# farshid83/dpsvm

Measured on AMD Instinct MI355X. Metric: wall-clock training time (s) to tol=1e-3, MNIST even-odd RBF, at 1/2/4/8 MI355X, lower is better.
Workload: dtype fp32

## Files before the change

### dpsvm_amd/csrc/include/dpsvm/device_state.hpp

```cpp
#pragma once

#include <cstdint>

namespace dpsvm {

constexpr int kNQ = 16;
constexpr int kStepRows = 128;
constexpr int kStepThreads = 256;
constexpr int kFinThreads = 1024;
constexpr int kRowsKC = 1008;

enum CacheMode : int32_t {
  kCacheDense = 0,
  kCacheLRU = 1,
};

enum RowOp : int32_t {
  kOpCompute = 0,
  kOpFetch = 1,
};

enum DoneCode : int32_t {
  kRunning = 0,
  kConverged = 1,
// ... 64 lines not shown
      if (r.when(f)) return *out = r.kind, true;
  return false;
}

inline int ws_new_auto(int ws_new, int q, int dp) {
  const int n = ws_new > 0 ? (ws_new < q ? ws_new : q) : (dp >= 128 ? q : 3 * q / 4);
  return n > 2 ? n : 2;
}

struct alignas(16) SmoCtrl {
  int32_t iter;
  int32_t done;
  int32_t final_applied;
  int32_t nq;
  int32_t i_hi, i_lo;
  int32_t line_hi, line_lo;
  float c_hi, c_lo;
  float b_hi, b_lo;
  int32_t n_compute;
  int32_t n_spill;
  int32_t q_idx[kNQ];
  int32_t q_line[kNQ];
  int32_t q_op[kNQ];
  int32_t q_hsrc[kNQ];
  int32_t q_hspill[kNQ];
  float q_sq[kNQ];
  const float* q_ptr[kNQ];
  int32_t hand, hhand, pad0, pad1;
  int64_t hits, misses, rows_computed, x_passes, spec_rows, host_hits, spills;
};

struct alignas(16) SmoStatus {
  int64_t iter;
  int32_t done;
  int32_t seq;
  float b_hi, b_lo;
  int64_t hits, misses, rows_computed, x_passes, spec_rows, host_hits, spills;
  int64_t outer;
  int64_t ws_p1_round;
  int32_t ws_p, ws_damped;
  float nu_ext[4];
};

struct alignas(16) CandRecord {
  uint64_t key_hi, key_lo;
};

struct alignas(16) FusedRec {
  int32_t i_hi, i_lo;
  float a_hi, a_lo;
  int32_t iter, done;
  float b_hi, b_lo;
};
struct alignas(16) FusedCacheRec {
  int32_t i_hi, i_lo;
  float a_hi, a_lo;
  int32_t iter, done;
  float b_hi, b_lo;
  int32_t n_new;
  int32_t hand0, span;
  int32_t hand;
  int32_t hit_line[2];
  int32_t hhand, pad0;
  int32_t line[kNQ];
  int32_t key[kNQ];
  int32_t old[kNQ];
  int32_t hline[kNQ];
  int32_t hold[kNQ];
  int64_t hits, misses, rows_computed, x_passes, spec_rows, host_hits, spills;
};

constexpr int kFusedThreads = 256;
constexpr int kStatusEvery = 32;

struct SmoArgs {
  const float* x;
  const float* xsq;
  const float* y;
  float* alpha;
  float* f;
  float* lines;
  int64_t ldl;
  int32_t* slot_of;
  int32_t* key_of;
  uint8_t* ref;
  float* hlines;
  int32_t* hslot_of;
  int32_t* hkey_of;
  int32_t H;
  uint64_t* partials;
  SmoCtrl* ctrl;
  SmoStatus* status;
  const uint8_t* records;
  uint8_t* my_record;
  int64_t rec_bytes;
  int64_t n, nl, off;
  int64_t x_row0;
  int32_t d, dp, G, L;
  int32_t world;
  int32_t cache_mode;
  int32_t partitioned;
  int32_t spec;
  int32_t clip;
  float C, gamma, eps, tau;
  int64_t max_iter;
  int32_t fused_rows;
  int32_t fused_G;
  uint64_t* stamps;
  int32_t* plru_meta;
  int64_t plru_stride;
  uint64_t* const* xpeer;
  int32_t xrank, xworld;
  int32_t xstride;
  int32_t xpoll_kb;
  int32_t xpoll_sleep;
  int64_t xtimeout_ticks;
  int32_t* census;
  int64_t census_ticks;
  int32_t eta_gram;
};
constexpr int kXchGranules = 4;

constexpr int kWsMax = 192;
constexpr int kWsCand = 16;
constexpr int kWsCandStd = 8;
constexpr int kWsCand1 = 4;
constexpr int kWsSelThreads = 256;
constexpr int kWsMaxGroups = 256;
constexpr int kWsListsPerThread = 4;
constexpr int kWsMaxRPT = 32;
constexpr int kWsSolveThreads = 1024;
constexpr int64_t kWsAutoRows = 50000;
constexpr int kWsMaxBlocks = 128;
constexpr int kWsAutoBlocks = 32;
constexpr int kWsAutoUnion = 16 * kWsMax;
constexpr int kWsMaxAll = 32 * kWsMax;
constexpr int kWsCacheWindow = 512;

inline int64_t ws_cache_min_lines(int q_max) { return 2 * (int64_t)q_max + kWsCacheWindow; }
constexpr int kWsWindowMulti = 8192;
inline int64_t ws_cache_multi_min_lines(int blocks, int q) { return 2 * (int64_t)blocks * q + kWsWindowMulti; }

inline int64_t production_line_cap(int64_t cache_lines, int ws_q, int engines) {
  if (cache_lines <= 0 || engines != 0) return cache_lines;
  const int64_t lo = ws_cache_min_lines(ws_q);
  return cache_lines < lo ? lo : cache_lines;
}
constexpr int kWsMergeThreads = 1024;
constexpr int kWsMaxPass1Splits = 16;
constexpr int kWsPass1Cols = 1024;
constexpr int64_t kWsAutoBlocksRows = 50000;
constexpr int64_t kWsSwitchRounds = 32;

struct alignas(16) WsCtrl {
  int64_t iter;
  int64_t outer;
  int32_t done;
  int32_t n_apply;
  int32_t q[2];
  float b_hi, b_lo;
  int32_t nonfinite;
  int32_t n_miss;
  int32_t hand;
  int32_t solve_cnt;
  int32_t rank_cnt;
  int32_t pad[1];
  int32_t idx[2][kWsMaxAll];
  int32_t line[2][kWsMaxAll];
  int32_t apply_idx[kWsMaxAll];
  int32_t apply_line[kWsMaxAll];
  float apply_coef[kWsMaxAll];
  int32_t miss_row[kWsMaxAll], miss_line[kWsMaxAll];
  int64_t rows_computed, row_hits;
  int32_t uidx[2][kWsMaxAll];
  int32_t uq[2];
  int32_t qb[2][kWsMaxBlocks];
  int32_t nab[kWsMaxBlocks];
  int32_t inb[kWsMaxBlocks];
  int32_t badb[kWsMaxBlocks];
  int32_t pad2[3];
  float t_last;
  int32_t n_damped;
  int32_t p_act;
  int32_t p_round;
  int32_t clipb[kWsMaxBlocks];
  int64_t p1_round;
  int32_t nu_cls;
  int32_t pad3[3];
  float nu_ext[4];
};

struct WsArgs {
  const float* gram;
  int64_t ldg;
  const float* y;
  float* alpha;
  float* f;
  int64_t n, nl, off;
  int32_t G, rpt;
  int32_t world;
  int32_t G_all;
  int32_t q_max, n_new, inner_max;
  float rel_local;
  float eps_floor;
  float C, eps, tau;
  int32_t clip;
  int64_t max_iter;
  int32_t cache;
  int32_t L;
  int32_t* slot_of;
  int32_t* key_of;
  uint64_t* cand_out;
  uint64_t* cand;
  float* subg;
  float* aux;
  WsCtrl* ctrl;
  SmoStatus* status;
  uint64_t* stamps;
  uint64_t* const* xpeer;
  int32_t xrank;
  int32_t xcw;
  int64_t xsub;
  int64_t xsub_rows;
  int64_t xpart;
  int64_t xtimeout_ticks;
  int32_t blocks;
  float* dfs;
  float* dalpha;
  double* part;
  int32_t rank;
  int32_t aux_stride;
  int32_t wss;
  float t_halve;
  int32_t clip_fallback;
  int32_t ks;
  int32_t p1G;
  uint64_t* sorted;
  int32_t direct_sub;
  int32_t ncand;
  const float* c_row;
  int64_t fold;
  int32_t diag;
  int32_t nu_mode;
};
constexpr int ws_ncand(int ncand) { return ncand > 0 && ncand < kWsCand ? ncand : kWsCand; }
constexpr int64_t ws_xch_words(int64_t G_all, int64_t q_max) {
  return 2 * G_all * 4 * kWsCand1 + 2 * q_max * (q_max + 1);
}
constexpr int64_t ws_xch_cand_words_multi(int64_t G_all) { return 2 * G_all * 4 * kWsCand; }
constexpr int64_t ws_xch_part_words(int64_t P1_all, int64_t ks) { return 2 * P1_all * ks * 4; }
constexpr int64_t ws_xch_sub_words(int64_t P, int64_t q, int64_t q1) {
  return 2 * ((P * q * (q + 1)) > (q1 * (q1 + 1)) ? P * q * (q + 1) : q1 * (q1 + 1));
}
constexpr int64_t ws_xch_words_multi(int64_t G_all, int64_t P1_all, int64_t ks, int64_t P, int64_t q, int64_t q1) {
  return ws_xch_cand_words_multi(G_all) + ws_xch_part_words(P1_all, ks) + ws_xch_sub_words(P, q, q1);
}
constexpr int kStampRing = 4096;
constexpr int kStampSlots = 12;

}
```

### dpsvm_amd/csrc/kernels/ws_common.hpp

```cpp
#pragma once

#include <hip/hip_runtime.h>

#include "dpsvm/common.hpp"
#include "dpsvm/device_state.hpp"
#include "device_util.hpp"
#include "xch.hpp"

namespace dpsvm {
namespace dev {

constexpr int kWsGatherThreads = 256;
constexpr int kWsMaxCand = kWsMaxGroups * kWsCand1;
constexpr int kWsHash = 1024;

#define WS_STAMP(k)                                                                            \
  do {                                                                                         \
    if (a.stamps) a.stamps[(size_t)(c->outer % kStampRing) * 2 * kStampSlots + (k)] =          \
        __builtin_amdgcn_s_memrealtime();                                                      \
  } while (0)

__device__ __forceinline__ float f_add1(float fj, float c, float k) {
#pragma clang fp contract(off)
  return fj + c * k;
// ... 83 lines not shown
  return bin;
}

__device__ __forceinline__ uint64_t block_scan_fields(uint64_t v, uint64_t* wsum, uint64_t* total) {
  const int lane = threadIdx.x & 63, wave = threadIdx.x >> 6;
  const uint64_t below = (1ull << lane) - 1ull;
  uint64_t pre = 0, wtot = 0;
#pragma unroll
  for (int f = 0; f < 4; ++f) {
#pragma unroll
    for (int b = 0; b < 3; ++b) {
      const int bit = 12 * f + b;
      const uint64_t mk = __ballot((v >> bit) & 1);
      pre += (uint64_t)__popcll(mk & below) << bit;
      wtot += (uint64_t)__popcll(mk) << bit;
    }
  }
  if (lane == 0) wsum[wave] = wtot;
  __syncthreads();
  uint64_t off = 0, tot = 0;
#pragma unroll
  for (int w = 0; w < kWsGatherThreads / 64; ++w) {
    off += w < wave ? wsum[w] : 0;
    tot += wsum[w];
  }
  *total = tot;
  __syncthreads();
  return off + pre;
}

__device__ __forceinline__ uint32_t ws_hash(int32_t idx) { return ((uint32_t)idx * 2654435761u) >> 22; }

__device__ __forceinline__ void ws_hash_insert(int32_t* keys, int32_t* vals, int32_t idx, int32_t v) {
  uint32_t h = ws_hash(idx);
  while (true) {
    const int32_t old = atomicCAS(keys + h, -1, idx);
    if (old == -1) {
      vals[h] = v;
      return;
    }
    h = (h + 1) & (kWsHash - 1);
  }
}

__device__ __forceinline__ int32_t ws_hash_find(const int32_t* keys, const int32_t* vals, int32_t idx) {
  uint32_t h = ws_hash(idx);
  for (int probe = 0; probe < kWsHash; ++probe) {
    const int32_t k = keys[h];
    if (k == idx) return vals[h];
    if (k == -1) return -1;
    h = (h + 1) & (kWsHash - 1);
  }
  return -1;
}

__device__ __forceinline__ void ws_status(SmoStatus* s, const WsCtrl* c) {
  if (!s) return;
  s->iter = c->iter;
  s->done = c->done;
  s->b_hi = c->b_hi;
  s->b_lo = c->b_lo;
  s->outer = c->outer;
  s->rows_computed = c->rows_computed;
  s->misses = c->rows_computed;
  s->hits = c->row_hits;
  s->ws_p1_round = c->p1_round;
  s->ws_p = c->p_act;
  s->ws_damped = c->n_damped;
  __atomic_store_n(&s->seq, (int32_t)c->outer, __ATOMIC_RELEASE);
}

__device__ __forceinline__ int64_t ws_xcand(const WsArgs& a, int par, int slot) {
  return ((int64_t)par * a.G_all + slot) * a.xcw;
}

__device__ __forceinline__ int64_t ws_xrow(const WsArgs& a, int par, int row) {
  return a.xsub + ((int64_t)par * a.xsub_rows + row) * (a.q_max + 1);
}

__device__ __forceinline__ int64_t ws_nparts(const WsArgs& a) {
  return (int64_t)a.world * a.p1G * max(1, a.ks);
}
__device__ __forceinline__ int64_t ws_xpart(const WsArgs& a, int par, int64_t k) {
  return a.xpart + ((int64_t)par * ws_nparts(a) + k) * 4;
}

__device__ __forceinline__ bool ws_tag_ok(uint64_t g, uint64_t t) { return (g >> 48) == (t >> 48); }

__device__ __forceinline__ void ws_put64(uint64_t* dst, uint64_t t, uint64_t v) {
  xch_store<true>(dst, t | (v >> 16));
  xch_store<true>(dst + 1, t | (v & 0xffffull));
}
__device__ __forceinline__ uint64_t ws_get64(uint64_t g0, uint64_t g1) {
  return ((g0 & ((1ull << 48) - 1)) << 16) | (g1 & 0xffffull);
}

template <int N>
__device__ __forceinline__ bool ws_poll(const WsArgs& a, const uint64_t* g, uint64_t t, uint64_t (&out)[N]) {
  const uint64_t t0 = __builtin_amdgcn_s_memrealtime();
  while (true) {
#pragma unroll
    for (int i = 0; i < N; ++i) out[i] = xch_load<true>(g + i);
    bool all = true;
#pragma unroll
    for (int i = 0; i < N; ++i) all &= ws_tag_ok(out[i], t);
    if (all) return true;
    if ((int64_t)(__builtin_amdgcn_s_memrealtime() - t0) > a.xtimeout_ticks) return false;
    __builtin_amdgcn_s_sleep(1);
  }
}

__device__ __forceinline__ void ws_cx(uint64_t& x, uint64_t& y) {
  const uint64_t lo = x < y ? x : y, hi = x < y ? y : x;
  x = lo;
  y = hi;
}

__device__ __forceinline__ void ws_top4_merge(uint64_t (&a)[kWsCand1], const uint64_t (&b)[kWsCand1]) {
  static_assert(kWsCand1 == 4, "4-entry bitonic merge");
#pragma unroll
  for (int i = 0; i < 4; ++i) a[i] = a[i] < b[3 - i] ? a[i] : b[3 - i];
  ws_cx(a[0], a[2]);
  ws_cx(a[1], a[3]);
  ws_cx(a[0], a[1]);
  ws_cx(a[2], a[3]);
}

__device__ __forceinline__ void ws_comm_fail(const WsArgs& a, WsCtrl* c) {
  if (threadIdx.x == 0) {
    c->done = kCommFail;
    c->n_apply = 0;
    ws_status(a.status, c);
  }
}

__device__ __forceinline__ void ws_comm_fail_thread(const WsArgs& a, WsCtrl* c) {
  c->done = kCommFail;
  c->n_apply = 0;
  ws_status(a.status, c);
}

__device__ __forceinline__ double wave_sum_f64(double v) {
#pragma unroll
  for (int o = 32; o > 0; o >>= 1) v += __shfl_xor(v, o);
  return v;
}

constexpr float kWsTFull = 0.9f;

__device__ __forceinline__ float ws_line_search(const WsArgs& a, int P) {
  if (P <= 1) return 1.f;
  const int lane = threadIdx.x & 63;
  double q = 0.0, g = 0.0;
  for (int k = lane; k < ws_nparts(a); k += 64) {
    q += a.part[2 * k];
    g += a.part[2 * k + 1];
  }
  q = wave_sum_f64(q);
  g = wave_sum_f64(g);
  if (!(g > 0.0)) return 0.f;
  if (!(q > g)) return 1.f;
  const float t = (float)(g / q);
  return t >= kWsTFull ? 1.f : t;
}

}
}
```

### dpsvm_amd/csrc/kernels/ws_merge.hip

```cpp
#include <hip/hip_runtime.h>

#include <cstdlib>
#include <string>

#include "dpsvm/common.hpp"
#include "dpsvm/device_state.hpp"
#include "device_util.hpp"
#include "kernels.hpp"
#include "ws_common.hpp"
#include "ws_merge.hpp"
#include "../runtime/hip_check.hpp"

namespace dpsvm {
namespace dev {

template <bool kFold = false>
__device__ __forceinline__ void ws_gather_row(const WsArgs& a, WsCtrl* c, const int32_t* s_idx, int q, int ra,
                                              const float* line, int xr) {
  const int tid = threadIdx.x;
  float* dst = a.subg + (size_t)ra * a.q_max;
  if (ra >= q) {
    for (int b = tid; b < a.q_max; b += kWsGatherThreads) dst[b] = 0.f;
    if (tid == 0) a.aux[ra] = 0.f;
    return;
// ... 178 lines not shown
  for (int w = 0; w < kWsMergeThreads / 64; ++w) {
    off += w < wave ? wsum[w] : 0;
    tot += wsum[w];
  }
  *total = tot;
  __syncthreads();
  return off + pre;
}

template <int X>
__device__ __forceinline__ int multi_scan_merge(const int (&v)[X], int (&slot)[X], int* msum, int nact) {
  constexpr int NW = kWsMergeThreads / 64;
  const int lane = threadIdx.x & 63, wave = threadIdx.x >> 6;
  const uint64_t below = (1ull << lane) - 1ull;
  int pre[X];
#pragma unroll
  for (int x = 0; x < X; ++x) {
    pre[x] = 0;
    if (x < nact) {
      int wt = 0;
#pragma unroll
      for (int b = 0; b < 2; ++b) {
        const uint64_t m = __ballot((v[x] >> b) & 1);
        pre[x] += __popcll(m & below) << b;
        wt += __popcll(m) << b;
      }
      if (lane == 0) msum[x * NW + wave] = wt;
    }
  }
  __syncthreads();
  int base = 0;
#pragma unroll
  for (int x = 0; x < X; ++x) {
    slot[x] = base;
    if (x < nact) {
      int off = 0, tot = 0;
#pragma unroll
      for (int w = 0; w < NW; ++w) {
        const int t = msum[x * NW + w];
        off += w < wave ? t : 0;
        tot += t;
      }
      slot[x] = base + off + pre[x];
      base += tot;
    }
  }
  return base;
}

constexpr int kMH = 8192;
static_assert(kMH == 8192, "11-bit bucket hash");
constexpr int kMHB = kMH / 4;
typedef int mh_i4 __attribute__((ext_vector_type(4)));
__device__ __forceinline__ uint32_t mh_bucket(int32_t idx) { return ((uint32_t)idx * 2654435761u) >> 21; }
__device__ __forceinline__ void mh_insert(int32_t* keys, uint16_t* vals, int32_t idx, int32_t v) {
  uint32_t b = mh_bucket(idx);
  while (true) {
    const mh_i4 kb = *(const mh_i4*)(keys + 4 * b);
    const int s = kb.x == -1 ? 0 : kb.y == -1 ? 1 : kb.z == -1 ? 2 : kb.w == -1 ? 3 : 4;
    if (s == 4) {
      b = (b + 1) & (kMHB - 1);
      continue;
    }
    if (atomicCAS(keys + 4 * b + s, -1, idx) == -1) {
      vals[4 * b + s] = (uint16_t)v;
      return;
    }
  }
}
template <int N>
__device__ __forceinline__ void mh_insert_n(int32_t* keys, uint16_t* vals, const int32_t (&idx)[N],
                                            const int32_t (&v)[N]) {
  uint32_t b[N];
  mh_i4 kb[N];
#pragma unroll
  for (int j = 0; j < N; ++j) {
    b[j] = mh_bucket(idx[j] < 0 ? 0 : idx[j]);
    if (idx[j] >= 0) kb[j] = *(const mh_i4*)(keys + 4 * b[j]);
  }
  int sl[N];
  bool won[N];
#pragma unroll
  for (int j = 0; j < N; ++j) {
    sl[j] = kb[j].x == -1 ? 0 : kb[j].y == -1 ? 1 : kb[j].z == -1 ? 2 : kb[j].w == -1 ? 3 : 4;
    won[j] = false;
    if (idx[j] >= 0 && sl[j] < 4) won[j] = atomicCAS(keys + 4 * b[j] + sl[j], -1, idx[j]) == -1;
  }
#pragma unroll
  for (int j = 0; j < N; ++j) {
    if (idx[j] < 0) continue;
    if (won[j]) vals[4 * b[j] + sl[j]] = (uint16_t)v[j];
    else mh_insert(keys, vals, idx[j], v[j]);
  }
}

__device__ __forceinline__ int32_t mh_find_from(const int32_t* keys, const uint16_t* vals, int32_t idx, uint32_t b) {
  for (int probe = 0; probe < kMHB; ++probe) {
    const mh_i4 kb = *(const mh_i4*)(keys + 4 * b);
    const int s = kb.x == idx ? 0 : kb.y == idx ? 1 : kb.z == idx ? 2 : kb.w == idx ? 3 : -1;
    if (s >= 0) return (int32_t)vals[4 * b + s];
    if (kb.w == -1) return -1;
    b = (b + 1) & (kMHB - 1);
  }
  return -1;
}
__device__ __forceinline__ int32_t mh_find(const int32_t* keys, const uint16_t* vals, int32_t idx) {
  return mh_find_from(keys, vals, idx, mh_bucket(idx));
}

template <int N>
__device__ __forceinline__ void mh_find_n(const int32_t* keys, const uint16_t* vals, const int32_t (&idx)[N],
                                          int32_t (&out)[N]) {
  uint32_t b[N];
  mh_i4 kb[N];
#pragma unroll
  for (int j = 0; j < N; ++j) {
    b[j] = mh_bucket(idx[j] < 0 ? 0 : idx[j]);
    if (idx[j] >= 0) kb[j] = *(const mh_i4*)(keys + 4 * b[j]);
  }
#pragma unroll
  for (int j = 0; j < N; ++j) {
    out[j] = -1;
    if (idx[j] < 0) continue;
    const int32_t k = idx[j];
    const int s = kb[j].x == k ? 0 : kb[j].y == k ? 1 : kb[j].z == k ? 2 : kb[j].w == k ? 3 : -1;
    if (s >= 0) out[j] = (int32_t)vals[4 * b[j] + s];
    else if (kb[j].w != -1) out[j] = mh_find_from(keys, vals, k, (b[j] + 1) & (kMHB - 1));
  }
}

constexpr int kXCollectThreads = 256;
__global__ __launch_bounds__(kXCollectThreads) void ws_xcollect_cand_kernel(WsArgs a) {
  WsCtrl* c = a.ctrl;
  if (c->done != kRunning) return;
  if (blockIdx.x == 0 && threadIdx.x == 0) WS_STAMP(15);
  const int e = (int)(blockIdx.x * kXCollectThreads + threadIdx.x);
  const int nk = a.blocks > 1 ? ws_ncand(a.ncand) : kWsCand1;
  bool ok = true;
  if (e < a.G_all * 2 * kWsCand) {
    const int l = e / (2 * kWsCand), side = (e / kWsCand) & 1, r = e % kWsCand;
    if (r < nk) {
      uint64_t g[2];
      ok = ws_poll<2>(a, a.xpeer[a.xrank] + ws_xcand(a, (int)(c->outer & 1), l) + side * (a.xcw / 2) + 2 * r,
                      xtag((uint32_t)c->outer + 1u), g);
      a.cand[e] = ok ? ws_get64(g[0], g[1]) : kKeyNone;
    } else {
      a.cand[e] = kKeyNone;
    }
  }
  if (!ok) ws_comm_fail_thread(a, c);
  if (blockIdx.x == 0 && threadIdx.x == 0) WS_STAMP(16);
}

struct RankLds {
  uint64_t k[kWsMaxGroups * kWsCand];
  int real[kWsMergeThreads / 64];
};
constexpr int kRankGroups = kWsMaxGroups * kWsCand * 16 / kWsMergeThreads;
__device__ __forceinline__ void ws_rank_body(const WsArgs& a, RankLds& L) {
  constexpr int T = kWsMergeThreads;
  constexpr int NK = kWsMaxGroups * kWsCand, CH = kRankGroups;
  constexpr int KPW = NK / CH, SUB = T / KPW, PAIRS = NK / (2 * SUB);
  static_assert(NK % CH == 0 && T % KPW == 0 && SUB == 16 && NK % (2 * SUB) == 0, "rank geometry");
  uint64_t* const s_k = L.k;
  int* const s_real = L.real;
  const WsCtrl* c = a.ctrl;
  const int side = blockIdx.x / CH, chunk = blockIdx.x % CH, tid = threadIdx.x;
  if (blockIdx.x == 0 && tid == 0) WS_STAMP(21);
  const int G = a.G_all;
  int real = 0;
  {
    constexpr int PER = NK / T;
    static_assert(NK % T == 0, "rank load geometry");
    uint64_t kk[PER];
#pragma unroll
    for (int j = 0; j < PER; ++j) {
      const int e = tid + j * T, l = e / kWsCand, r = e % kWsCand;
      kk[j] = l < G ? a.cand[(size_t)l * 2 * kWsCand + side * kWsCand + r] : kKeyNone;
    }
#pragma unroll
    for (int j = 0; j < PER; ++j) {
      s_k[tid + j * T] = kk[j];
      real += kk[j] != kKeyNone ? 1 : 0;
    }
  }
#pragma unroll
  for (int o = 32; o > 0; o >>= 1) real += __shfl_xor(real, o);
  if ((tid & 63) == 0) s_real[tid >> 6] = real;
  __syncthreads();
  int n_real = 0;
#pragma unroll
  for (int w = 0; w < T / 64; ++w) n_real += s_real[w];
  const int e = chunk * KPW + tid / SUB, sub = tid % SUB;
  const uint64_t k = s_k[e];
  int cnt = 0;
#pragma unroll 8
  for (int i = 0; i < PAIRS; ++i) {
    const int e2 = 2 * (sub + SUB * i);
    cnt += (s_k[e2] < k ? 1 : 0) + (s_k[e2 + 1] < k ? 1 : 0);
  }
#pragma unroll
  for (int o = 1; o < SUB; o <<= 1) cnt += __shfl_xor(cnt, o);
  uint64_t* out = a.sorted + (size_t)side * NK;
  auto put = [&](int i, uint64_t v) {
    __hip_atomic_store(out + i, v, __ATOMIC_RELAXED, __HIP_MEMORY_SCOPE_AGENT);
  };
  if (sub == 0 && k != kKeyNone) put(cnt, k);
  if (tid < KPW && chunk * KPW + tid >= n_real) put(chunk * KPW + tid, kKeyNone);
}

struct MergeLds {
  __attribute__((aligned(16))) int32_t hk[2][kMH];
  uint16_t hv[2][kMH];
  int32_t keep[kWsMaxAll + 2];
  int32_t idx[kWsMaxAll];
  int wsum[kWsMergeThreads / 64];
  int msum[(kWsMaxGroups * kWsCand / kWsMergeThreads) * (kWsMergeThreads / 64)];
};
__device__ __forceinline__ void ws_merge_multi_body(const WsArgs& a, MergeLds& L) {
  constexpr int T = kWsMergeThreads;
  constexpr int NK = kWsMaxGroups * kWsCand;
  constexpr int X = NK / T;
  constexpr int U = kWsMaxAll / T;
  static_assert(NK % T == 0 && kWsMaxAll % T == 0 && U <= 7, "previous union: <= 7 rows per thread (3-bit scans)");
  static_assert(kMH == kWsWindowMulti && kWsWindowMulti == 8 * T && NK <= 65536,
                "cache mode: the CLOCK window's pins alias the low side's key table; 16-bit ranks");
  auto& s_hk = L.hk;
  auto& s_hv = L.hv;
  int32_t* const s_keep = L.keep;
  int32_t* const s_idx = L.idx;
  int* const s_wsum = L.wsum;
  int* const s_msum = L.msum;
  WsCtrl* c = a.ctrl;
  const int tid = threadIdx.x;
  const bool lead = tid == 0;
  if (lead) WS_STAMP(1);
  const int par = (int)(c->outer & 1);
  const int P = max(1, min(c->p_act, a.blocks)), Qmax = P * a.q_max;
  const int q_prev = c->uq[par ^ 1];
  const int want = q_prev == 0 ? Qmax : min(P * a.n_new, Qmax);
  int32_t pidx[U];
#pragma unroll
  for (int h = 0; h < U; ++h) pidx[h] = U * tid + h < q_prev ? c->uidx[par ^ 1][U * tid + h] : -1;
  uint64_t v[2][X];
  auto ld_sorted = [&](int i) -> uint64_t {
    return __hip_atomic_load(a.sorted + i, __ATOMIC_RELAXED, __HIP_MEMORY_SCOPE_AGENT);
  };
#pragma unroll
  for (int x = 0; x < X; ++x) {
    v[0][x] = ld_sorted(tid + x * T);
    v[1][x] = ld_sorted(NK + tid + x * T);
  }
  const uint64_t gu = ld_sorted(0), gl = ld_sorted(NK);
  for (int t = tid; t < 2 * kMH; t += T) (&s_hk[0][0])[t] = -1;
  if (lead) WS_STAMP(20);
  __syncthreads();
  if (lead) WS_STAMP(11);
  const float b_hi = key_value(gu), b_lo = -key_value(gl);
  const int64_t it0 = c->iter;
  int stop = kRunning;
  if (c->nonfinite) stop = kNonFinite;
  else if (gu == kKeyNone || gl == kKeyNone) stop = kNoPair;
  else if (!isfinite(b_hi) || !isfinite(b_lo)) stop = kNonFinite;
  else if (!(b_lo > b_hi + 2.0f * a.eps)) stop = kConverged;
  else if (it0 >= a.max_iter) stop = kMaxIter;
  if (stop != kRunning) {
    if (lead) {
      c->done = stop;
      c->n_apply = 0;
      c->b_hi = b_hi;
      c->b_lo = b_lo;
      ws_status(a.status, c);
    }
    return;
  }
  int32_t* hk_u = s_hk[0];
  uint16_t* hv_u = s_hv[0];
  int32_t* hk_l = s_hk[1];
  uint16_t* hv_l = s_hv[1];
  int32_t* const s_line = s_hk[0] + kMH / 2;
  const int half = (want + 1) / 2;
  uint64_t ku[X], kl[X];
  int32_t iu[X], il[X], er[X];
#pragma unroll
  for (int x = 0; x < X; ++x) {
    const int e = tid + x * T;
    ku[x] = e < half ? v[0][x] : kKeyNone;
    kl[x] = e < half ? v[1][x] : kKeyNone;
    iu[x] = ku[x] != kKeyNone ? (int32_t)key_index(ku[x]) : -1;
    il[x] = kl[x] != kKeyNone ? (int32_t)key_index(kl[x]) : -1;
    er[x] = e;
  }
  mh_insert_n<X>(hk_u, hv_u, iu, er);
  mh_insert_n<X>(hk_l, hv_l, il, er);
  __syncthreads();
  if (lead) WS_STAMP(12);
  bool kpu[X], kpl[X];
  {
    int32_t rl[X], ru[X];
    mh_find_n<X>(hk_l, hv_l, iu, rl);
    mh_find_n<X>(hk_u, hv_u, il, ru);
#pragma unroll
    for (int x = 0; x < X; ++x) {
      const int e = tid + x * T;
      kpu[x] = iu[x] >= 0 && !(rl[x] >= 0 && rl[x] < e);
      kpl[x] = il[x] >= 0 && !(ru[x] >= 0 && ru[x] <= e);
    }
  }
  int cnt[X], slot[X];
#pragma unroll
  for (int x = 0; x < X; ++x) cnt[x] = (int)kpu[x] + (int)kpl[x];
  const int kept = multi_scan_merge<X>(cnt, slot, s_msum, min(X, (half + T - 1) / T));
  const int n_chosen = min(kept, want);
#pragma unroll
  for (int x = 0; x < X; ++x) {
    const int e = tid + x * T;
    if (e < half) {
      const int su = slot[x], sl = su + (int)kpu[x];
      const bool cu = kpu[x] && su < want, cl = kpl[x] && sl < want;
      s_keep[2 * e] = cu ? su : -1;
      s_keep[2 * e + 1] = cl ? sl : -1;
      if (cu) s_idx[su] = (int32_t)key_index(ku[x]);
      if (cl) s_idx[sl] = (int32_t)key_index(kl[x]);
    }
  }
  __syncthreads();
  if (lead) WS_STAMP(13);
  bool pk[U];
  int npk = 0;
#pragma unroll
  for (int h = 0; h < U; ++h) pk[h] = false;
  if (n_chosen < Qmax) {
    int32_t ru[U], rl[U];
    mh_find_n<U>(hk_u, hv_u, pidx, ru);
    mh_find_n<U>(hk_l, hv_l, pidx, rl);
#pragma unroll
    for (int h = 0; h < U; ++h)
      pk[h] = pidx[h] >= 0 && !((ru[h] >= 0 && s_keep[2 * ru[h]] >= 0) || (rl[h] >= 0 && s_keep[2 * rl[h] + 1] >= 0));
  }
#pragma unroll
  for (int h = 0; h < U; ++h) npk += (int)pk[h];
  int ptotal = 0;
  if (n_chosen < Qmax) {
    int at = n_chosen + block_scan_merge<3>(npk, s_wsum, &ptotal);
#pragma unroll
    for (int h = 0; h < U; ++h) {
      if (pk[h]) {
        if (at < Qmax) s_idx[at] = pidx[h];
        ++at;
      }
    }
  }
  const int Q = min(Qmax, n_chosen + ptotal);
  __syncthreads();
  if (lead) WS_STAMP(14);
  if (a.cache) {
    int32_t* s_pin = s_hk[1];
    int32_t* s_victim = s_hk[0];
    const int L = a.L, hand = c->hand;
    const int W = min(L, kWsWindowMulti);
    for (int w = tid; w < kWsWindowMulti; w += T) s_pin[w] = 0;
    __syncthreads();
    int32_t ln[U];
#pragma unroll
    for (int h = 0; h < U; ++h) {
      ln[h] = -1;
      const int u = tid + h * T;
      if (u < Q) {
        ln[h] = a.slot_of[s_idx[u]];
        if (ln[h] >= 0) {
          const int o = (ln[h] - hand + L) % L;
          if (o < W) s_pin[o] = 1;
        }
      }
    }
    __syncthreads();
    int mrank[U], n_miss = 0;
#pragma unroll
    for (int h = 0; h < U; ++h) {
      mrank[h] = n_miss;
      if (h * T < Q) {
        const bool mh = tid + h * T < Q && ln[h] < 0;
        int tot = 0;
        mrank[h] = n_miss + block_scan_merge<1>((int)mh, s_wsum, &tot);
        n_miss += tot;
      }
    }
    constexpr int SPT = kWsWindowMulti / T;
    bool fr[SPT];
    int nf = 0;
#pragma unroll
    for (int k = 0; k < SPT; ++k) {
      fr[k] = SPT * tid + k < W && !s_pin[SPT * tid + k];
      nf += (int)fr[k];
    }
    int n_free = 0;
    const int frank = block_scan_merge<4>(nf, s_wsum, &n_free);
    int at = frank, last_used = -1;
#pragma unroll
    for (int k = 0; k < SPT; ++k) {
      if (fr[k]) {
        if (at < n_miss) {
          s_victim[at] = (hand + SPT * tid + k) % L;
          last_used = SPT * tid + k;
        }
        ++at;
      }
    }
    __syncthreads();
    if (last_used >= 0 && frank < n_miss && at >= n_miss) c->hand = (hand + last_used + 1) % L;
#pragma unroll
    for (int h = 0; h < U; ++h) {
      const int u = tid + h * T;
      if (u < Q && ln[h] < 0) {
        const int r = mrank[h];
        const int32_t row = s_idx[u];
        const int32_t vl = s_victim[r];
        const int32_t old = a.key_of[vl];
        if (old >= 0) a.slot_of[old] = -1;
        a.key_of[vl] = row;
        a.slot_of[row] = vl;
        c->miss_row[r] = row;
        c->miss_line[r] = vl;
        ln[h] = vl;
      }
      if (u < Q) s_line[u] = ln[h];
    }
    if (lead) {
      c->n_miss = n_miss;
      c->rows_computed += n_miss;
      c->row_hits += Q - n_miss;
    }
    __syncthreads();
  }
  const bool pow2 = (P & (P - 1)) == 0;
  const int lg = pow2 ? __ffs(P) - 1 : 0;
  for (int u = tid; u < Q; u += T) {
    const int32_t row = s_idx[u];
    c->uidx[par][u] = row;
    const int pi = u >> 1;
    const int b = pow2 ? pi & (P - 1) : pi % P, la = 2 * (pow2 ? pi >> lg : pi / P) + (u & 1);
    c->idx[par][b * a.q_max + la] = row;
    c->line[par][b * a.q_max + la] = a.cache ? s_line[u] : row;
  }
  if (tid < a.blocks) {
    const int NP = (Q + 1) >> 1, b = tid;
    const int cnt = b < P && b < NP ? (NP - 1 - b) / P + 1 : 0;
    const int last = b + P * (cnt - 1);
    c->qb[par][b] = cnt == 0 ? 0 : 2 * (cnt - 1) + ((last == NP - 1 && (Q & 1)) ? 1 : 2);
  }
  if (lead) {
    c->uq[par] = Q;
    c->q[par] = Q;
    c->p_round = P;
    c->b_hi = b_hi;
    c->b_lo = b_lo;
    WS_STAMP(2);
  }
}

__global__ __launch_bounds__(kWsMergeThreads) void ws_rank_merge_kernel(WsArgs a) {
  __shared__ union {
    RankLds r;
    MergeLds m;
  } L;
  __shared__ int s_last;
  WsCtrl* c = a.ctrl;
  if (c->done != kRunning) {
    if (blockIdx.x == 0 && threadIdx.x == 0) c->n_apply = 0;
    return;
  }
  ws_rank_body(a, L.r);
  asm volatile("s_waitcnt vmcnt(0)" ::: "memory");
  __syncthreads();
  if (threadIdx.x == 0)
    s_last = __hip_atomic_fetch_add(&c->rank_cnt, 1, __ATOMIC_RELAXED, __HIP_MEMORY_SCOPE_AGENT) ==
                     (int)gridDim.x - 1 ? 1 : 0;
  __syncthreads();
  if (!s_last) return;
  if (threadIdx.x == 0) c->rank_cnt = 0;
  ws_merge_multi_body(a, L.m);
}


__global__ __launch_bounds__(kWsGatherThreads) void ws_gather_multi_kernel(WsArgs a) {
  __shared__ int32_t s_idx[kWsMax];
  WsCtrl* c = a.ctrl;
  if (c->done != kRunning) return;
  const int tid = threadIdx.x;
  if (tid == 0 && blockIdx.x == 0) WS_STAMP(9);
  const int par = (int)(c->outer & 1);
  const int p = (int)blockIdx.x / a.q_max, ra = (int)blockIdx.x % a.q_max;
  const int q = c->qb[par][p];
  WsArgs b = a;
  b.subg = a.subg + (size_t)p * a.q_max * a.q_max;
  b.aux = a.aux + (size_t)p * kWsMax;
  if (a.xpeer != nullptr && ra >= q) return;
  if (ra >= q) {
    ws_gather_row(b, c, s_idx, q, ra, nullptr, p * a.q_max + ra);
    return;
  }
  for (int t = tid; t < q; t += kWsGatherThreads) s_idx[t] = c->idx[par][p * a.q_max + t];
  __syncthreads();
  const int64_t line = a.cache ? (int64_t)c->line[par][p * a.q_max + ra] : (int64_t)s_idx[ra];
  ws_gather_row(b, c, s_idx, q, ra, a.gram + line * a.ldg, p * a.q_max + ra);
  if (tid == 0 && blockIdx.x == 0) WS_STAMP(8);
}

__global__ __launch_bounds__(256) void ws_to_single_kernel(WsArgs a) {
  WsCtrl* c = a.ctrl;
  const int pp = (int)((c->outer + 1) & 1);
  const int q = min(c->uq[pp], a.q_max);
  for (int i = threadIdx.x; i < q; i += blockDim.x) c->idx[pp][i] = c->uidx[pp][i];
  if (threadIdx.x == 0) c->q[pp] = q;
}

__global__ __launch_bounds__(256) void ws_pack_rows_kernel(const float* __restrict__ x, int64_t off, int64_t nl,
                                                           int dp, const float* __restrict__ xsq,
                                                           const WsCtrl* __restrict__ c, float* __restrict__ out,
                                                           float* __restrict__ out_sq) {
  const int i = blockIdx.x;
  const int m = c->n_miss;
  const int64_t row = i < m ? (int64_t)c->miss_row[i] : -1;
  const bool own = row >= off && row < off + nl;
  f4* dst = (f4*)(out + (size_t)i * dp);
  const f4* src = (const f4*)(x + (size_t)(own ? row - off : 0) * dp);
  const f4 z = {0.f, 0.f, 0.f, 0.f};
  for (int k = threadIdx.x; k < dp / 4; k += blockDim.x) dst[k] = own ? src[k] : z;
  if (threadIdx.x == 0) out_sq[i] = row >= 0 ? xsq[row] : 0.f;
}

}

namespace launch {

void ws_xcollect_cand(const WsArgs& a, hipStream_t s) {
  const int keys = a.G_all * 2 * kWsCand;
  dev::ws_xcollect_cand_kernel<<<dim3((unsigned)((keys + dev::kXCollectThreads - 1) / dev::kXCollectThreads)),
                                 dev::kXCollectThreads, 0, s>>>(a);
  post_launch("ws_xcollect_cand", s);
}

void ws_merge_multi(const WsArgs& a, hipStream_t s) {
  DPSVM_CHECK(a.fold == 0, "ws_merge_multi: multi-block rounds are not implemented for regression (fold)");
  DPSVM_CHECK(a.nu_mode == 0, "ws_merge_multi: multi-block rounds are not implemented for the nu duals (nu_mode)");
  DPSVM_CHECK(a.blocks > 1 && a.blocks <= kWsMaxBlocks && a.blocks * a.q_max <= kWsMaxAll && a.G_all <= kWsMaxGroups && a.q_max % 2 == 0 &&
                  (!a.cache || (ws_cache_multi_supported(a.L, a.blocks, a.q_max) && a.blocks * a.q_max <= dev::kMH / 2)),
              "ws_merge_multi: multi-block rounds need <= 256 candidate lists, an even q_max and "
              "(cache mode) <= 4096 union rows and L >= 2 P q_max + 4096 lines");
  DPSVM_CHECK(a.sorted != nullptr, "ws_merge_multi: no sort buffer");
  DPSVM_CHECK(!a.xpeer || a.xcw >= 4 * kWsCand, "ws_merge_multi: peer exchange slots too narrow");
  dev::ws_rank_merge_kernel<<<2 * dev::kRankGroups, kWsMergeThreads, 0, s>>>(a);
  post_launch("ws_rank_merge", s);
}

void ws_gather(const WsArgs& a, hipStream_t s) {
  if (a.fold > 0) {
    DPSVM_CHECK(a.blocks == 1 && !a.cache && a.world == 1 && a.xpeer == nullptr && a.off == 0 && a.n == 2 * a.fold &&
                    a.nl == a.n && a.ldg >= a.fold,
                "ws_gather: regression (fold) runs one-block rounds on the resident Gram, one rank");
    if (a.nu_mode) dev::ws_gather_kernel<true, true><<<dim3(a.q_max), dev::kWsGatherThreads, 0, s>>>(a);
    else dev::ws_gather_kernel<true><<<dim3(a.q_max), dev::kWsGatherThreads, 0, s>>>(a);
    post_launch("ws_gather_fold", s);
    return;
  }
  if (a.nu_mode) {
    DPSVM_CHECK(a.blocks == 1 && !a.cache && a.world == 1 && a.xpeer == nullptr && a.off == 0 && a.nl == a.n,
                "ws_gather: the nu duals run one-block rounds on the resident Gram, one rank");
    dev::ws_gather_kernel<false, true><<<dim3(a.q_max), dev::kWsGatherThreads, 0, s>>>(a);
    post_launch("ws_gather_nu", s);
    return;
  }
  if (a.blocks > 1) {
    dev::ws_gather_multi_kernel<<<dim3(a.blocks * a.q_max), dev::kWsGatherThreads, 0, s>>>(a);
    post_launch("ws_gather_multi", s);
  } else if (a.cache) {
    dev::ws_gather_lines_kernel<<<dim3(a.q_max), dev::kWsGatherThreads, 0, s>>>(a);
    post_launch("ws_gather_lines", s);
  } else {
    dev::ws_gather_kernel<false><<<dim3(a.q_max), dev::kWsGatherThreads, 0, s>>>(a);
    post_launch("ws_gather", s);
  }
}

void ws_merge(const WsArgs& a, hipStream_t s) {
  DPSVM_CHECK(a.fold == 0, "ws_merge: the kernel-row cache is not implemented for regression (fold)");
  DPSVM_CHECK(a.nu_mode == 0, "ws_merge: the kernel-row cache is not implemented for the nu duals (nu_mode)");
  dev::ws_merge_kernel<<<1, dev::kWsGatherThreads, 0, s>>>(a);
  post_launch("ws_merge", s);
}

void ws_to_single(const WsArgs& a, hipStream_t s) {
  dev::ws_to_single_kernel<<<1, 256, 0, s>>>(a);
  post_launch("ws_to_single", s);
}

void ws_pack_rows(const float* x, int64_t off, int64_t nl, int dp, const float* xsq, const WsCtrl* ctrl, int q_max,
                  float* out, float* out_sq, hipStream_t s) {
  DPSVM_CHECK(dp % 16 == 0, "ws_pack_rows: dp must be a multiple of 16");
  dev::ws_pack_rows_kernel<<<dim3(q_max), 256, 0, s>>>(x, off, nl, dp, xsq, ctrl, out, out_sq);
  post_launch("ws_pack_rows", s);
}

bool ws_cache_supported(int64_t L, int q_max) { return L >= ws_cache_min_lines(q_max); }

bool ws_cache_multi_supported(int64_t L, int blocks, int q_max) {
  return L >= ws_cache_multi_min_lines(blocks, q_max);
}

}
}
```

### dpsvm_amd/csrc/kernels/ws_solve.hip

```cpp
#include <hip/hip_runtime.h>

#include <atomic>

#include "dpsvm/common.hpp"
#include "dpsvm/device_state.hpp"
#include "device_util.hpp"
#include "kernels.hpp"
#include "ws_common.hpp"
#include "ws_solve.hpp"
#include "../runtime/hip_check.hpp"

namespace dpsvm {
namespace dev {

constexpr int kWsSolvePollBatch = 10;

template <bool kBox, bool kFull, bool kMulti, bool kW2, int NS = 3, bool kRowC = false, bool kDiag = false,
          bool kNu = false>
__global__ __launch_bounds__(kWsSolveThreads) void ws_solve_kernel(WsArgs a) {
  extern __shared__ __attribute__((aligned(16))) float K[];
  __shared__ float s_a[kWsMax + 128], s_y[kWsMax], s_f[kWsMax];
  __shared__ int32_t s_idx[kWsMax], s_line[kWsMax];
  __shared__ float s_c[kRowC ? kWsMax : 1];
  WsCtrl* c = a.ctrl;
  const int tid = threadIdx.x, lane = tid & 63, wave = tid >> 6;
  if (tid == 0) WS_STAMP(0);
  if (c->done != kRunning) return;
  const int par = (int)(c->outer & 1);
  const int blk = kMulti ? (int)blockIdx.x : 0;
  const int q = kMulti ? c->qb[par][blk] : c->q[par];
  const float b_hi = c->b_hi, b_lo = c->b_lo;
  const int64_t it0 = c->iter;
  const int ldk = a.q_max;
  const int ib = blk * a.q_max;
  const float* subg = a.subg + (size_t)blk * ldk * ldk;
  const float* aux = a.aux + (size_t)blk * kWsMax;
  bool xok = true;
  if (a.xpeer != nullptr) {
    const int64_t R = c->outer;
    const uint64_t t = xtag((uint32_t)R + 1u);
    const uint64_t* rows = a.xpeer[a.xrank] + ws_xrow(a, par, ib);
    const int w = ldk + 1, n_e = q * w;
    constexpr int kB = kWsSolvePollBatch;
    const uint64_t t0 = __builtin_amdgcn_s_memrealtime();
    for (int e0 = 0; e0 < n_e && xok; e0 += kB * kWsSolveThreads) {
      uint64_t v[kB];
      uint32_t need = 0;
#pragma unroll
      for (int k = 0; k < kB; ++k) {
        const int e = e0 + tid + k * kWsSolveThreads;
        const int col = e - (e / w) * w;
        const bool want = e < n_e && (col < q || col == ldk);
        v[k] = want ? xch_load<true>(rows + e) : t;
        need |= want ? 1u << k : 0u;
      }
      while (true) {
#pragma unroll
        for (int k = 0; k < kB; ++k)
          if (((need >> k) & 1u) && ws_tag_ok(v[k], t)) need &= ~(1u << k);
        if (need == 0) break;
        if ((int64_t)(__builtin_amdgcn_s_memrealtime() - t0) > a.xtimeout_ticks) {
          xok = false;
          break;
        }
        __builtin_amdgcn_s_sleep(1);
#pragma unroll
        for (int k = 0; k < kB; ++k)
          if ((need >> k) & 1u) v[k] = xch_load<true>(rows + e0 + tid + k * kWsSolveThreads);
      }
#pragma unroll
      for (int k = 0; k < kB; ++k) {
        const int e = e0 + tid + k * kWsSolveThreads;
        if (e >= n_e) break;
        const int ra = e / w, col = e - ra * w;
        if (col < ldk) K[ra * ldk + col] = col < q ? __uint_as_float((uint32_t)v[k]) : 0.f;
        else s_f[ra] = __uint_as_float((uint32_t)v[k]);
      }
    }
    if (tid < q) {
      s_a[tid] = aux[a.aux_stride + tid];
      s_y[tid] = aux[2 * a.aux_stride + tid];
      s_idx[tid] = c->idx[par][ib + tid];
      s_line[tid] = c->line[par][ib + tid];
      if constexpr (kRowC) s_c[tid] = a.c_row[c->idx[par][ib + tid]];
    }
  } else if (a.direct_sub) {
    int32_t gi = 0;
    if (tid < q) {
      gi = c->idx[par][ib + tid];
      s_idx[tid] = gi;
      s_line[tid] = c->line[par][ib + tid];
    }
    __syncthreads();
    float fv = 0.f, av = 0.f, yv = 0.f, cv = 0.f;
    if (tid < q) {
      fv = a.f[gi];
      av = a.alpha[gi];
      yv = a.y[gi];
      if constexpr (kRowC) cv = a.c_row[gi];
    }
    const int n = q * ldk;
    constexpr int U = 4;
    for (int e0 = tid; e0 < n; e0 += U * kWsSolveThreads) {
      float v[U];
#pragma unroll
      for (int u = 0; u < U; ++u) {
        const int e = e0 + u * kWsSolveThreads;
        const int ra = e / ldk, col = e - ra * ldk;
        v[u] = e < n && ra <= col && col < q ? a.gram[(int64_t)s_idx[ra] * a.ldg + s_idx[col]] : 0.f;
      }
#pragma unroll
      for (int u = 0; u < U; ++u) {
        const int e = e0 + u * kWsSolveThreads;
        const int ra = e / ldk, col = e - ra * ldk;
        if (e < n && ra <= col) {
          K[e] = v[u];
          if (col < q && col != ra) K[col * ldk + ra] = v[u];
        }
      }
    }
    if (tid < q) {
      s_f[tid] = fv;
      s_a[tid] = av;
      s_y[tid] = yv;
      if constexpr (kRowC) s_c[tid] = cv;
    }
  } else {
    const int n = q * ldk;
    if ((ldk & 3) == 0) {
      const f4* src = (const f4*)subg;
      f4* dst = (f4*)K;
      const int n4 = n >> 2;
      for (int e = tid; e < n4; e += 4 * kWsSolveThreads) {
        f4 v[4];
#pragma unroll
        for (int u = 0; u < 4; ++u) {
          const int k = e + u * kWsSolveThreads;
          v[u] = src[k < n4 ? k : 0];
        }
#pragma unroll
        for (int u = 0; u < 4; ++u)
          if (e + u * kWsSolveThreads < n4) dst[e + u * kWsSolveThreads] = v[u];
      }
    } else {
      for (int e = tid; e < n; e += kWsSolveThreads) K[e] = subg[e];
    }
    if (tid < q) {
      s_f[tid] = aux[tid];
      s_a[tid] = aux[a.aux_stride + tid];
      s_y[tid] = aux[2 * a.aux_stride + tid];
      s_idx[tid] = c->idx[par][ib + tid];
      s_line[tid] = c->line[par][ib + tid];
      if constexpr (kRowC) s_c[tid] = a.c_row[c->idx[par][ib + tid]];
    }
  }
  bool xfail = false;
  if (a.xpeer != nullptr) xfail = !__syncthreads_and(xok);
  else __syncthreads();
  if (xfail && tid == 0) ws_comm_fail_thread(a, c);
  if (tid == 0) WS_STAMP(3);
  if (wave != 0) return;

  if constexpr (kRowC)
    ws_solve_run<kBox, kFull, kMulti, kW2, NS, true, kDiag>(a, c, K, s_a, s_y, s_f, s_idx, s_line, q, blk, ib, it0,
                                                            b_hi, b_lo, xfail, s_c);
  else
    ws_solve_run<kBox, kFull, kMulti, kW2, NS, false, kDiag, kNu>(a, c, K, s_a, s_y, s_f, s_idx, s_line, q, blk, ib,
                                                                  it0, b_hi, b_lo, xfail);
}

}

namespace launch {

void ws_solve(const WsArgs& a, hipStream_t s) {
  const size_t lds = (size_t)a.q_max * a.q_max * sizeof(float);
  const bool box = a.clip == (int)ClipMode::Box, full = a.q_max == kWsMax, multi = a.blocks > 1, w2 = a.wss == 2;
  const bool rowc = a.c_row != nullptr;
  using Fn = void (*)(WsArgs);
#define WS_SOLVE_FNS(W2, RC)                                                                                     \
  dev::ws_solve_kernel<false, false, false, W2, 3, RC>, dev::ws_solve_kernel<false, true, false, W2, 3, RC>,    \
      dev::ws_solve_kernel<true, false, false, W2, 3, RC>, dev::ws_solve_kernel<true, true, false, W2, 3, RC>,  \
      dev::ws_solve_kernel<false, false, true, W2, 3, RC>, dev::ws_solve_kernel<false, true, true, W2, 3, RC>,  \
      dev::ws_solve_kernel<true, false, true, W2, 3, RC>, dev::ws_solve_kernel<true, true, true, W2, 3, RC>
  static const Fn fns[32] = {WS_SOLVE_FNS(false, false), WS_SOLVE_FNS(true, false), WS_SOLVE_FNS(false, true),
                             WS_SOLVE_FNS(true, true)};
#undef WS_SOLVE_FNS
#define WS_SOLVE_FNS2(W2, RC)                                                                                    \
  dev::ws_solve_kernel<false, false, false, W2, 2, RC>, dev::ws_solve_kernel<true, false, false, W2, 2, RC>,    \
      dev::ws_solve_kernel<false, false, true, W2, 2, RC>, dev::ws_solve_kernel<true, false, true, W2, 2, RC>
  static const Fn fns2[16] = {WS_SOLVE_FNS2(false, false), WS_SOLVE_FNS2(true, false), WS_SOLVE_FNS2(false, true),
                              WS_SOLVE_FNS2(true, true)};
#undef WS_SOLVE_FNS2
#define WS_SOLVE_FNS1(W2, RC)                                                                                    \
  dev::ws_solve_kernel<false, false, false, W2, 1, RC>, dev::ws_solve_kernel<true, false, false, W2, 1, RC>,    \
      dev::ws_solve_kernel<false, false, true, W2, 1, RC>, dev::ws_solve_kernel<true, false, true, W2, 1, RC>
  static const Fn fns1[16] = {WS_SOLVE_FNS1(false, false), WS_SOLVE_FNS1(true, false), WS_SOLVE_FNS1(false, true),
                              WS_SOLVE_FNS1(true, true)};
#undef WS_SOLVE_FNS1
  const int v = (rowc ? 16 : 0) + (w2 ? 8 : 0) + (multi ? 4 : 0) + (box ? 2 : 0) + (full ? 1 : 0);
  const int v2 = (rowc ? 8 : 0) + (w2 ? 4 : 0) + (multi ? 2 : 0) + (box ? 1 : 0);
  const bool one = a.q_max <= 64, two = !one && a.q_max <= 128;
#define WS_SOLVE_FNSD(NS_, FULL)                                                                                   \
  dev::ws_solve_kernel<true, FULL, false, false, NS_, false, true>,                                                \
      dev::ws_solve_kernel<true, FULL, false, true, NS_, false, true>,                                             \
      dev::ws_solve_kernel<true, FULL, false, false, NS_, true, true>,                                             \
      dev::ws_solve_kernel<true, FULL, false, true, NS_, true, true>
  static const Fn fnsd[16] = {WS_SOLVE_FNSD(3, false), WS_SOLVE_FNSD(3, true), WS_SOLVE_FNSD(2, false),
                              WS_SOLVE_FNSD(1, false)};
#undef WS_SOLVE_FNSD
  const bool diag = a.diag != 0;
  DPSVM_CHECK(!diag || (box && !multi), "ws_solve: the general-diagonal kernels run one block with box clipping");
  const int vd = (one ? 12 : two ? 8 : full ? 4 : 0) + (rowc ? 2 : 0) + (w2 ? 1 : 0);
#define WS_SOLVE_FNSN(NS_, FULL)                                                                                   \
  dev::ws_solve_kernel<true, FULL, false, false, NS_, false, false, true>,                                         \
      dev::ws_solve_kernel<true, FULL, false, true, NS_, false, false, true>,                                      \
      dev::ws_solve_kernel<true, FULL, false, false, NS_, false, true, true>,                                      \
      dev::ws_solve_kernel<true, FULL, false, true, NS_, false, true, true>
  static const Fn fnsn[16] = {WS_SOLVE_FNSN(3, false), WS_SOLVE_FNSN(3, true), WS_SOLVE_FNSN(2, false),
                              WS_SOLVE_FNSN(1, false)};
#undef WS_SOLVE_FNSN
  const bool nu = a.nu_mode != 0;
  DPSVM_CHECK(!nu || (box && !multi && !rowc && a.xpeer == nullptr),
              "ws_solve: the nu duals run one block with box clipping and the scalar C, one rank");
  const int vn = (one ? 12 : two ? 8 : full ? 4 : 0) + (diag ? 2 : 0) + (w2 ? 1 : 0);
  const Fn fn = nu ? fnsn[vn] : diag ? fnsd[vd] : one ? fns1[v2] : two ? fns2[v2] : fns[v];
  static std::atomic<size_t> attr[kMaxDevices][64];
  static std::atomic<size_t> attr_d[kMaxDevices][16];
  static std::atomic<size_t> attr_n[kMaxDevices][16];
  std::atomic<size_t>& at = nu     ? attr_n[current_device()][vn]
                            : diag ? attr_d[current_device()][vd]
                                   : attr[current_device()][one ? 48 + v2 : two ? 32 + v2 : v];
  size_t cur = at.load(std::memory_order_relaxed);
  if (lds > 64 * 1024 && lds > cur) {
    HIP_CHECK(hipFuncSetAttribute((const void*)fn, hipFuncAttributeMaxDynamicSharedMemorySize, (int)lds));
    while (lds > cur && !at.compare_exchange_weak(cur, lds)) {
    }
  }
  fn<<<multi ? a.blocks : 1, kWsSolveThreads, lds, s>>>(a);
  post_launch("ws_solve", s);
}

}
}
```

Before: 0.01514.

## Pack per-block solve header and cut dependent control loads across WS kernels

The merge kernel now writes a per-block record (q, parity, b_hi, b_lo) so that solve blocks on the direct sub-Gram path read one 16-byte struct and prefetch both parity index rows before checking done, instead of issuing a chain of dependent control loads. The rank step pads its LDS key lists and replaces the linear pairwise count with a per-list binary search, and the partition reduction is unrolled to overlap loads. Merge hoists its control reads and vectorises hash-table initialisation. A new host check restricts direct sub-Gram loads to single-rank multi-block runs without a cache, and s_line now takes the row index itself, which assumes line equals index in that mode.

Result: faster. 0.01497 (median of 6 runs) (-1.1%).

```diff
diff --git a/dpsvm_amd/csrc/include/dpsvm/device_state.hpp b/dpsvm_amd/csrc/include/dpsvm/device_state.hpp
--- a/dpsvm_amd/csrc/include/dpsvm/device_state.hpp
+++ b/dpsvm_amd/csrc/include/dpsvm/device_state.hpp
@@ -240,6 +240,12 @@
 constexpr int64_t kWsAutoBlocksRows = 50000;
 constexpr int64_t kWsSwitchRounds = 32;
 
+struct alignas(16) WsBlockRec {
+  int32_t q;
+  int32_t par;
+  float b_hi, b_lo;
+};
+
 struct alignas(16) WsCtrl {
   int64_t iter;
   int64_t outer;
@@ -276,6 +282,7 @@
   int32_t nu_cls;
   int32_t pad3[3];
   float nu_ext[4];
+  WsBlockRec brec[kWsMaxBlocks];
 };
 
 struct WsArgs {
diff --git a/dpsvm_amd/csrc/kernels/ws_common.hpp b/dpsvm_amd/csrc/kernels/ws_common.hpp
--- a/dpsvm_amd/csrc/kernels/ws_common.hpp
+++ b/dpsvm_amd/csrc/kernels/ws_common.hpp
@@ -259,9 +259,23 @@
   if (P <= 1) return 1.f;
   const int lane = threadIdx.x & 63;
   double q = 0.0, g = 0.0;
-  for (int k = lane; k < ws_nparts(a); k += 64) {
-    q += a.part[2 * k];
-    g += a.part[2 * k + 1];
+  constexpr int B = 4;
+  const int64_t np = ws_nparts(a);
+  for (int64_t k0 = lane; k0 < np; k0 += 64 * B) {
+    double vq[B], vg[B];
+#pragma unroll
+    for (int u = 0; u < B; ++u) {
+      const int64_t k = k0 + 64 * u < np ? k0 + 64 * u : k0;
+      vq[u] = a.part[2 * k];
+      vg[u] = a.part[2 * k + 1];
+    }
+#pragma unroll
+    for (int u = 0; u < B; ++u) {
+      if (k0 + 64 * u < np) {
+        q += vq[u];
+        g += vg[u];
+      }
+    }
   }
   q = wave_sum_f64(q);
   g = wave_sum_f64(g);
diff --git a/dpsvm_amd/csrc/kernels/ws_merge.hip b/dpsvm_amd/csrc/kernels/ws_merge.hip
--- a/dpsvm_amd/csrc/kernels/ws_merge.hip
+++ b/dpsvm_amd/csrc/kernels/ws_merge.hip
@@ -354,16 +354,18 @@
   if (blockIdx.x == 0 && threadIdx.x == 0) WS_STAMP(16);
 }
 
+constexpr int kRankStride = kWsCand + 1;
 struct RankLds {
-  uint64_t k[kWsMaxGroups * kWsCand];
+  uint64_t k[kWsMaxGroups * kRankStride];
   int real[kWsMergeThreads / 64];
 };
 constexpr int kRankGroups = kWsMaxGroups * kWsCand * 16 / kWsMergeThreads;
 __device__ __forceinline__ void ws_rank_body(const WsArgs& a, RankLds& L) {
   constexpr int T = kWsMergeThreads;
   constexpr int NK = kWsMaxGroups * kWsCand, CH = kRankGroups;
-  constexpr int KPW = NK / CH, SUB = T / KPW, PAIRS = NK / (2 * SUB);
-  static_assert(NK % CH == 0 && T % KPW == 0 && SUB == 16 && NK % (2 * SUB) == 0, "rank geometry");
+  constexpr int KPW = NK / CH, SUB = T / KPW, LPT = kWsMaxGroups / SUB;
+  static_assert(NK % CH == 0 && T % KPW == 0 && SUB == 16 && kWsMaxGroups % SUB == 0 && kWsCand == 16,
+                "rank geometry: 16 threads a key, a 16-key list searched in four halvings and one compare");
   uint64_t* const s_k = L.k;
   int* const s_real = L.real;
   const WsCtrl* c = a.ctrl;
@@ -382,7 +384,8 @@
     }
 #pragma unroll
     for (int j = 0; j < PER; ++j) {
-      s_k[tid + j * T] = kk[j];
+      const int e = tid + j * T;
+      s_k[(e / kWsCand) * kRankStride + e % kWsCand] = kk[j];
       real += kk[j] != kKeyNone ? 1 : 0;
     }
   }
@@ -394,13 +397,18 @@
 #pragma unroll
   for (int w = 0; w < T / 64; ++w) n_real += s_real[w];
   const int e = chunk * KPW + tid / SUB, sub = tid % SUB;
-  const uint64_t k = s_k[e];
+  const uint64_t k = s_k[(e / kWsCand) * kRankStride + e % kWsCand];
+  int lb[LPT];
+#pragma unroll
+  for (int i = 0; i < LPT; ++i) lb[i] = s_k[(sub + SUB * i) * kRankStride + 7] < k ? 8 : 0;
+#pragma unroll
+  for (int h = 4; h > 0; h >>= 1) {
+#pragma unroll
+    for (int i = 0; i < LPT; ++i) lb[i] += s_k[(sub + SUB * i) * kRankStride + lb[i] + h - 1] < k ? h : 0;
+  }
   int cnt = 0;
-#pragma unroll 8
-  for (int i = 0; i < PAIRS; ++i) {
-    const int e2 = 2 * (sub + SUB * i);
-    cnt += (s_k[e2] < k ? 1 : 0) + (s_k[e2 + 1] < k ? 1 : 0);
-  }
+#pragma unroll
+  for (int i = 0; i < LPT; ++i) cnt += lb[i] + (s_k[(sub + SUB * i) * kRankStride + kWsCand - 1] < k ? 1 : 0);
 #pragma unroll
   for (int o = 1; o < SUB; o <<= 1) cnt += __shfl_xor(cnt, o);
   uint64_t* out = a.sorted + (size_t)side * NK;
@@ -437,13 +445,8 @@
   const int tid = threadIdx.x;
   const bool lead = tid == 0;
   if (lead) WS_STAMP(1);
-  const int par = (int)(c->outer & 1);
-  const int P = max(1, min(c->p_act, a.blocks)), Qmax = P * a.q_max;
-  const int q_prev = c->uq[par ^ 1];
-  const int want = q_prev == 0 ? Qmax : min(P * a.n_new, Qmax);
-  int32_t pidx[U];
-#pragma unroll
-  for (int h = 0; h < U; ++h) pidx[h] = U * tid + h < q_prev ? c->uidx[par ^ 1][U * tid + h] : -1;
+  const int64_t outer = c->outer, it0 = c->iter;
+  const int p_act = c->p_act, nonfinite = c->nonfinite, uq0 = c->uq[0], uq1 = c->uq[1];
   uint64_t v[2][X];
   auto ld_sorted = [&](int i) -> uint64_t {
     return __hip_atomic_load(a.sorted + i, __ATOMIC_RELAXED, __HIP_MEMORY_SCOPE_AGENT);
@@ -454,14 +457,23 @@
     v[1][x] = ld_sorted(NK + tid + x * T);
   }
   const uint64_t gu = ld_sorted(0), gl = ld_sorted(NK);
-  for (int t = tid; t < 2 * kMH; t += T) (&s_hk[0][0])[t] = -1;
+  {
+    const mh_i4 none = {-1, -1, -1, -1};
+    for (int t = tid; t < 2 * kMH / 4; t += T) ((mh_i4*)&s_hk[0][0])[t] = none;
+  }
+  const int par = (int)(outer & 1);
+  const int P = max(1, min(p_act, a.blocks)), Qmax = P * a.q_max;
+  const int q_prev = par ? uq0 : uq1;
+  const int want = q_prev == 0 ? Qmax : min(P * a.n_new, Qmax);
+  int32_t pidx[U];
+#pragma unroll
+  for (int h = 0; h < U; ++h) pidx[h] = U * tid + h < q_prev ? c->uidx[par ^ 1][U * tid + h] : -1;
   if (lead) WS_STAMP(20);
   __syncthreads();
   if (lead) WS_STAMP(11);
   const float b_hi = key_value(gu), b_lo = -key_value(gl);
-  const int64_t it0 = c->iter;
   int stop = kRunning;
-  if (c->nonfinite) stop = kNonFinite;
+  if (nonfinite) stop = kNonFinite;
   else if (gu == kKeyNone || gl == kKeyNone) stop = kNoPair;
   else if (!isfinite(b_hi) || !isfinite(b_lo)) stop = kNonFinite;
   else if (!(b_lo > b_hi + 2.0f * a.eps)) stop = kConverged;
@@ -649,7 +661,9 @@
     const int NP = (Q + 1) >> 1, b = tid;
     const int cnt = b < P && b < NP ? (NP - 1 - b) / P + 1 : 0;
     const int last = b + P * (cnt - 1);
-    c->qb[par][b] = cnt == 0 ? 0 : 2 * (cnt - 1) + ((last == NP - 1 && (Q & 1)) ? 1 : 2);
+    const int qv = cnt == 0 ? 0 : 2 * (cnt - 1) + ((last == NP - 1 && (Q & 1)) ? 1 : 2);
+    c->qb[par][b] = qv;
+    c->brec[b] = WsBlockRec{qv, par, b_hi, b_lo};
   }
   if (lead) {
     c->uq[par] = Q;
@@ -680,7 +694,7 @@
                      (int)gridDim.x - 1 ? 1 : 0;
   __syncthreads();
   if (!s_last) return;
-  if (threadIdx.x == 0) c->rank_cnt = 0;
+  if (threadIdx.x == 0) __hip_atomic_store(&c->rank_cnt, 0, __ATOMIC_RELAXED, __HIP_MEMORY_SCOPE_AGENT);
   ws_merge_multi_body(a, L.m);
 }
 
diff --git a/dpsvm_amd/csrc/kernels/ws_solve.hip b/dpsvm_amd/csrc/kernels/ws_solve.hip
--- a/dpsvm_amd/csrc/kernels/ws_solve.hip
+++ b/dpsvm_amd/csrc/kernels/ws_solve.hip
@@ -25,14 +25,25 @@
   WsCtrl* c = a.ctrl;
   const int tid = threadIdx.x, lane = tid & 63, wave = tid >> 6;
   if (tid == 0) WS_STAMP(0);
-  if (c->done != kRunning) return;
-  const int par = (int)(c->outer & 1);
   const int blk = kMulti ? (int)blockIdx.x : 0;
-  const int q = kMulti ? c->qb[par][blk] : c->q[par];
-  const float b_hi = c->b_hi, b_lo = c->b_lo;
-  const int64_t it0 = c->iter;
   const int ldk = a.q_max;
   const int ib = blk * a.q_max;
+  const bool direct = a.direct_sub && a.xpeer == nullptr;
+  WsBlockRec rec = {0, 0, 0.f, 0.f};
+  int32_t row0 = 0, row1 = 0;
+  if (direct) {
+    rec = c->brec[blk];
+    if (tid < ldk) {
+      row0 = c->idx[0][ib + tid];
+      row1 = c->idx[1][ib + tid];
+    }
+  }
+  const int done = c->done;
+  const int64_t it0 = c->iter;
+  if (done != kRunning) return;
+  const int par = direct ? rec.par : (int)(c->outer & 1);
+  const int q = direct ? rec.q : kMulti ? c->qb[par][blk] : c->q[par];
+  const float b_hi = direct ? rec.b_hi : c->b_hi, b_lo = direct ? rec.b_lo : c->b_lo;
   const float* subg = a.subg + (size_t)blk * ldk * ldk;
   const float* aux = a.aux + (size_t)blk * kWsMax;
   bool xok = true;
@@ -84,12 +95,12 @@
       s_line[tid] = c->line[par][ib + tid];
       if constexpr (kRowC) s_c[tid] = a.c_row[c->idx[par][ib + tid]];
     }
-  } else if (a.direct_sub) {
+  } else if (direct) {
     int32_t gi = 0;
     if (tid < q) {
-      gi = c->idx[par][ib + tid];
+      gi = par ? row1 : row0;
       s_idx[tid] = gi;
-      s_line[tid] = c->line[par][ib + tid];
+      s_line[tid] = gi;
     }
     __syncthreads();
     float fv = 0.f, av = 0.f, yv = 0.f, cv = 0.f;
@@ -177,6 +188,8 @@
   const size_t lds = (size_t)a.q_max * a.q_max * sizeof(float);
   const bool box = a.clip == (int)ClipMode::Box, full = a.q_max == kWsMax, multi = a.blocks > 1, w2 = a.wss == 2;
   const bool rowc = a.c_row != nullptr;
+  DPSVM_CHECK(!a.direct_sub || (multi && !a.cache && a.world == 1),
+              "ws_solve: direct sub-Gram loads belong to multi-block rounds on the resident Gram, one rank");
   using Fn = void (*)(WsArgs);
 #define WS_SOLVE_FNS(W2, RC)                                                                                     \
   dev::ws_solve_kernel<false, false, false, W2, 3, RC>, dev::ws_solve_kernel<false, true, false, W2, 3, RC>,    \
```
